# Crispy13/GeneFuseRust

Measured on NVIDIA B200. Metric: read_pairs_per_sec_matched, higher is better.
Workload: dtype u8/int64

## Files before the change

### genefuserust_b200/csrc/gf_device.cuh

```cuda
#pragma once
#include <cuda_runtime.h>
#include <stdint.h>

#define GF_GENE_PAD 2304u
#define GF_EMPTY_VAL 0xFFFFFFFFu
#define GF_HASH_MULT 0x9E3779B1u
#define GF_KIND_UNIQUE 0u
#define GF_KIND_NORMAL 1u
#define GF_KIND_HIGH 2u
#define GF_SITE_STRAND (1u << 29)
#define GF_SITE_GOFF_MASK ((1u << 29) - 1u)
#define GF_MAX_GOFF (1u << 29)
#define GF_MAX_DUPES 7

struct GfDevIndex {
    const uint4* table;
    const uint32_t* dupes;
    const uint8_t* gene_ascii;
    const uint32_t* gene_start;
    const uint32_t* gene_len;
    const uint8_t* gene_rev;
    const uint16_t* granule_contig;
    const uint32_t* g_if;
    const uint32_t* g_ir;
    const unsigned long long* filter;
    uint32_t filter_words;
    const unsigned long long* filter_multi;
    uint32_t filter_multi_words;
    uint32_t n_genes;
    uint32_t max_sites;
    uint32_t bucket_shift;
    uint32_t bucket_mask;
    int32_t major_req, minor_req, mismatch_thr, deletion_thr;
};

__device__ __forceinline__ bool gf_is_acgt_upper(uint32_t c) {
    return ((c & 0xE0u) == 0x40u) && ((0x0010008Au >> (c & 31u)) & 1u);
}
__device__ __forceinline__ uint32_t gf_code_lo(uint32_t c) { return (c >> 2) & 1u; }
__device__ __forceinline__ uint32_t gf_code_hi(uint32_t c) { return (c >> 1) & 1u; }

// ... 54 lines not shown
            c.w == GF_EMPTY_VAL;
    return v;
}
__device__ __forceinline__ uint32_t gf_table_find(const GfDevIndex& ix, uint32_t key) {
    uint32_t b = gf_home_bucket(key, ix.bucket_shift);
    for (;;) {
        uint4 a, c;
        gf_load_bucket(ix.table, b, a, c);
        bool stop;
        uint32_t v = gf_match_bucket(a, c, key, &stop);
        if (stop) return v;
        b = (b + 1) & ix.bucket_mask;
    }
}

__device__ __forceinline__ uint32_t gf_filter_word(uint32_t key, uint32_t n_words) {
    return (uint32_t)(((unsigned long long)(key * GF_HASH_MULT) * n_words) >> 32);
}
__device__ __forceinline__ void gf_filter_masks(uint32_t key, uint32_t* any_lo, uint32_t* any_hi) {
    const uint32_t g1 = key * 0xC2B2AE35u, g2 = key * 0x27D4EB2Fu;
    *any_lo = (1u << (g1 >> 27)) | (1u << ((g1 >> 22) & 31u));
    *any_hi = (1u << (g2 >> 27)) | (1u << ((g2 >> 22) & 31u));
}
__device__ __forceinline__ uint32_t gf_multi_word(uint32_t key, uint32_t n_words) {
    return (uint32_t)(((unsigned long long)(key * 0x85EBCA6Bu) * n_words) >> 32);
}
__device__ __forceinline__ unsigned long long gf_multi_mask(uint32_t key) {
    const uint32_t g = key * 0x165667B1u;
    return (1ull << (g >> 26)) | (1ull << ((g >> 20) & 63u)) | (1ull << ((g >> 14) & 63u)) | (1ull << ((g >> 8) & 63u));
}
__device__ __forceinline__ uint32_t gf_filter_sites(const GfDevIndex& ix, unsigned long long w, uint32_t key, uint32_t max_sites) {
    uint32_t al, ah;
// ... 36 lines not shown
```

### genefuserust_b200/csrc/gf_index.cu

```cuda
#include <algorithm>
#include <chrono>
#include <cstdio>
#include <cstdlib>
#include <cstring>

#include "gf_internal.h"

namespace {

constexpr int SCAN_THREADS = 256;
constexpr int SCAN_ITEMS = 8;
constexpr int SCAN_TILE = SCAN_THREADS * SCAN_ITEMS;

__global__ void k_scan_reduce(const uint32_t* __restrict__ in, uint64_t n, uint32_t* __restrict__ block_sums) {
    __shared__ uint32_t warp_sums[SCAN_THREADS / 32];
    uint64_t base = (uint64_t)blockIdx.x * SCAN_TILE;
    uint32_t s = 0;
    for (int k = 0; k < SCAN_ITEMS; k++) {
        uint64_t i = base + (uint64_t)k * SCAN_THREADS + threadIdx.x;
        if (i < n) s += in[i];
    }
    for (int o = 16; o > 0; o >>= 1) s += __shfl_down_sync(0xFFFFFFFFu, s, o);
    if ((threadIdx.x & 31) == 0) warp_sums[threadIdx.x >> 5] = s;
    __syncthreads();
// ... 170 lines not shown
    bool head = i == 0 || (uint32_t)(items[i] >> 32) != (uint32_t)(items[i - 1] >> 32);
    uint32_t c = 0;
    if (head) {
        uint32_t len = run_len_capped(items, n, i, thr + 1);
        atomicAdd(&stats[0], 1ull);
        if (len == 1) atomicAdd(&stats[1], 1ull);
        else if (len <= thr) { atomicAdd(&stats[2], 1ull); c = len; }
        else atomicAdd(&stats[3], 1ull);
    }
    ncnt[i] = c;
}
__global__ void k_build_table(const unsigned long long* __restrict__ items, uint64_t n, uint32_t thr,
                              const uint32_t* __restrict__ dupe_off, uint32_t* __restrict__ dupes,
                              unsigned long long* __restrict__ table, uint32_t bucket_shift, uint32_t bucket_mask,
                              unsigned int* __restrict__ max_disp, unsigned long long* __restrict__ filter,
                              uint32_t filter_words, unsigned long long* __restrict__ filter_multi,
                              uint32_t filter_multi_words) {
    uint64_t i = (uint64_t)blockIdx.x * blockDim.x + threadIdx.x;
    if (i >= n) return;
    uint32_t key = (uint32_t)(items[i] >> 32);
    bool head = i == 0 || key != (uint32_t)(items[i - 1] >> 32);
    if (!head) return;
    uint32_t len = run_len_capped(items, n, i, thr + 1);
    uint32_t val;
    if (len == 1) {
        val = (GF_KIND_UNIQUE << 30) | (uint32_t)(items[i] & 0x3FFFFFFFull);
    } else if (len <= thr) {
        uint32_t off = dupe_off[i];
        for (uint32_t j = 0; j < len; j++) dupes[off + j] = (uint32_t)(items[i + j] & 0x3FFFFFFFull);
        val = (GF_KIND_NORMAL << 30) | (off << 3) | len;
    } else {
        val = (GF_KIND_HIGH << 30);
    }
    if (len <= thr) {
        uint32_t al, ah;
        gf_filter_masks(key, &al, &ah);
        atomicOr(filter + gf_filter_word(key, filter_words), ((unsigned long long)ah << 32) | al);
        if (len > 1) atomicOr(filter_multi + gf_multi_word(key, filter_multi_words), gf_multi_mask(key));
    }
    unsigned long long entry = ((unsigned long long)val << 32) | key;
    uint32_t b = gf_home_bucket(key, bucket_shift);
    uint32_t disp = 0;
    for (;;) {
        unsigned long long* slot = table + 4ull * b;
        bool done = false;
        for (int s = 0; s < 4 && !done; s++) {
            if (slot[s] == ~0ull) done = atomicCAS(slot + s, ~0ull, entry) == ~0ull;
        }
        if (done) break;
        b = (b + 1) & bucket_mask;
        disp++;
    }
// ... 110 lines not shown
};
struct BuildWorkspace {
    char* base = nullptr;
    size_t cap = 0, used = 0;
    ~BuildWorkspace() { if (base) cudaFree(base); }
    cudaError_t init(size_t bytes) { cap = bytes; return cudaMalloc((void**)&base, bytes); }
    template <class T>
    T* take(size_t n) {
        size_t bytes = (n * sizeof(T) + 255) & ~(size_t)255;
        if (used + bytes > cap) return nullptr;
        T* p = reinterpret_cast<T*>(base + used);
        used += bytes;
        return p;
    }
};
__global__ void k_interleave_planes(const uint32_t* __restrict__ pl, uint32_t stride, uint32_t* __restrict__ g_if,
                                    uint32_t* __restrict__ g_ir) {
    const uint32_t w = blockIdx.x * blockDim.x + threadIdx.x;
    if (w >= stride) return;
    const uint32_t lo = pl[w], hi = pl[(size_t)stride + w], v = pl[2ull * stride + w];
    uint4* f = reinterpret_cast<uint4*>(g_if + 8ull * w);
    uint4* r = reinterpret_cast<uint4*>(g_ir + 8ull * w);
    f[0] = make_uint4(lo, hi, v, pl[3ull * stride + w]);
    f[1] = make_uint4(pl[4ull * stride + w], pl[5ull * stride + w], 0u, 0u);
    r[0] = make_uint4(lo, hi, v, pl[6ull * stride + w]);
    r[1] = make_uint4(pl[7ull * stride + w], pl[8ull * stride + w], 0u, 0u);
}

}

int gf_build_index_device(gf_index* idx, const gf_gene_span* genes, uint32_t n_genes) {
    PhaseTimer pt;
    const uint32_t thr = (uint32_t)std::max(idx->params.skip_key_dup_threshold, 2);
    cudaStream_t st = idx->stream;

    idx->n_genes = n_genes;
    idx->gene_start.resize(n_genes);
    idx->gene_len.resize(n_genes);
    std::vector<uint8_t> rev(n_genes ? n_genes : 1, 0);
    uint64_t cur = GF_GENE_PAD, gene_bytes = 0;
    for (uint32_t g = 0; g < n_genes; g++) {
// ... 115 lines not shown
    }
    if (n_dupes >= (1u << 27)) {
        gf_set_error("too many NORMAL dupe sites for the 27-bit dupe offset");
        return GF_E_LIMIT;
    }

    pt.mark("classify");
    const uint64_t n_keys = h_stats[0];
    uint32_t bucket_bits = 6;
    while ((1ull << bucket_bits) * 2 < n_keys) bucket_bits++;
    const uint64_t n_buckets = 1ull << bucket_bits;
    GF_CUDA_TRY(cudaMalloc(&idx->d_table, n_buckets * 32));
    GF_CUDA_TRY(cudaMemsetAsync(idx->d_table, 0xFF, n_buckets * 32, st));
    GF_CUDA_TRY(cudaMalloc(&idx->d_dupes, sizeof(uint32_t) * ((size_t)n_dupes + 8)));
    unsigned int* d_maxdisp = (unsigned int*)(d_stats + 6);
    const int filter_bits = 8;
    const uint32_t filter_words = (uint32_t)std::max<uint64_t>(1024, (n_keys * (uint64_t)filter_bits + 63) / 64);
    const uint32_t filter_multi_words = (uint32_t)std::max<uint64_t>(1024, (h_stats[2] * 16 + 63) / 64);
    GF_CUDA_TRY(cudaMalloc(&idx->d_filter, sizeof(unsigned long long) * ((size_t)filter_words + filter_multi_words)));
    GF_CUDA_TRY(cudaMemsetAsync(idx->d_filter, 0, sizeof(unsigned long long) * ((size_t)filter_words + filter_multi_words), st));
    unsigned long long* d_filter_multi = (unsigned long long*)idx->d_filter + filter_words;
    if (n_items) {
        const unsigned cb = (unsigned)((n_items + 255) / 256);
        k_build_table<<<cb, 256, 0, st>>>(d_items, n_items, thr, d_doff, (uint32_t*)idx->d_dupes,
                                          (unsigned long long*)idx->d_table, 32 - bucket_bits,
                                          (uint32_t)(n_buckets - 1), d_maxdisp, (unsigned long long*)idx->d_filter,
                                          filter_words, d_filter_multi, filter_multi_words);
        GF_CUDA_TRY(cudaGetLastError());
    }
    unsigned int h_maxdisp = 0;
    GF_CUDA_TRY(cudaMemcpyAsync(&h_maxdisp, d_maxdisp, sizeof(unsigned int), cudaMemcpyDeviceToHost, st));
    GF_CUDA_TRY(cudaStreamSynchronize(st));

    pt.mark("table + filter");
    idx->dev.table = (const uint4*)idx->d_table;
    idx->dev.dupes = (const uint32_t*)idx->d_dupes;
    idx->dev.gene_ascii = (const uint8_t*)idx->d_gene_ascii;
    idx->dev.gene_start = (const uint32_t*)idx->d_gene_start;
    idx->dev.gene_len = (const uint32_t*)idx->d_gene_len;
    idx->dev.gene_rev = (const uint8_t*)idx->d_gene_rev;
    idx->dev.n_genes = n_genes;
    idx->dev.max_sites = thr;
    idx->dev.bucket_shift = 32 - bucket_bits;
    idx->dev.bucket_mask = (uint32_t)(n_buckets - 1);
    idx->dev.major_req = idx->params.major_gene_key_requirement;
    idx->dev.minor_req = idx->params.minor_gene_key_requirement;
    idx->dev.mismatch_thr = idx->params.mismatch_threshold;
    idx->dev.deletion_thr = idx->params.deletion_threshold;
    idx->dev.filter = (const unsigned long long*)idx->d_filter;
    idx->dev.filter_words = filter_words;
    idx->dev.filter_multi = d_filter_multi;
    idx->dev.filter_multi_words = filter_multi_words;

    const uint32_t n_pw = (uint32_t)((arena_len + 31) / 32);
    const size_t plane_stride = ((size_t)n_pw + 72 + 7) & ~(size_t)7;
    DevTmp tmp_planes;
    GF_CUDA_TRY(cudaMalloc(&tmp_planes.p, sizeof(uint32_t) * plane_stride * 9));
    GF_CUDA_TRY(cudaMemsetAsync(tmp_planes.p, 0, sizeof(uint32_t) * plane_stride * 9, st));
    GF_CUDA_TRY(cudaMalloc(&idx->d_planes, sizeof(uint32_t) * plane_stride * 16));
    uint32_t* pl = (uint32_t*)tmp_planes.p;
    uint32_t* gi = (uint32_t*)idx->d_planes;
    k_gene_planes<<<(n_pw + 255) / 256, 256, 0, st>>>((const uint8_t*)idx->d_gene_ascii, arena_len, n_pw, pl,
                                                      pl + plane_stride, pl + 2 * plane_stride);
    k_window_class<<<ex_blocks, EX_THREADS, 0, st>>>(idx->dev, (const uint8_t*)idx->d_gene_ascii, arena_len,
                                                     pl + 3 * plane_stride, pl + 6 * plane_stride,
                                                     (uint32_t)plane_stride);
    idx->dev.g_if = gi;
    idx->dev.g_ir = gi + 8 * plane_stride;
    k_interleave_planes<<<(unsigned)((plane_stride + 255) / 256), 256, 0, st>>>(pl, (uint32_t)plane_stride, gi, gi + 8 * plane_stride);
    GF_CUDA_TRY(cudaGetLastError());
    GF_CUDA_TRY(cudaEventRecord(e1, st));
    GF_CUDA_TRY(cudaStreamSynchronize(st));
    float ms = 0;
    GF_CUDA_TRY(cudaEventElapsedTime(&ms, e0, e1));

    pt.mark("gene planes + window class");
    gf_index_info& inf = idx->info;
    inf.n_sites = n_items;
    inf.n_keys = n_keys;
    inf.n_unique = h_stats[1];
    inf.n_normal = h_stats[2];
    inf.n_high = h_stats[3];
    inf.table_slots = n_buckets * 4;
    inf.table_bytes = n_buckets * 32;
    inf.max_displacement = h_maxdisp;
    inf.gene_bytes = gene_bytes;
    inf.device_bytes = n_buckets * 32 + sizeof(uint32_t) * ((size_t)n_dupes + 8) + arena_len + 9ull * (n_genes + 1) +
                       sizeof(uint32_t) * plane_stride * 16 + sizeof(unsigned long long) * ((size_t)filter_words + filter_multi_words);
    inf.build_ms = ms;
    return GF_OK;
}

int gf_lookup_device(gf_index* idx, const uint32_t* kmers, uint64_t n, gf_lookup* out) {
    if (n == 0) return GF_OK;
    DevTmp k, o;
    GF_CUDA_TRY(cudaMalloc(&k.p, sizeof(uint32_t) * n));
    GF_CUDA_TRY(cudaMalloc(&o.p, sizeof(gf_lookup) * n));
    GF_CUDA_TRY(cudaMemcpyAsync(k.p, kmers, sizeof(uint32_t) * n, cudaMemcpyHostToDevice, idx->stream));
    k_lookup<<<(unsigned)((n + 127) / 128), 128, 0, idx->stream>>>(idx->dev, (const uint32_t*)k.p, n, (gf_lookup*)o.p);
    GF_CUDA_TRY(cudaGetLastError());
    GF_CUDA_TRY(cudaMemcpyAsync(out, o.p, sizeof(gf_lookup) * n, cudaMemcpyDeviceToHost, idx->stream));
    GF_CUDA_TRY(cudaStreamSynchronize(idx->stream));
    return GF_OK;
// ... 2 lines not shown
```

### genefuserust_b200/csrc/gf_map.cu

```cuda
#include <climits>
#include <cstdlib>
#include <cstdio>

#include "gf_internal.h"
#include "gf_swar.cuh"

namespace {

#define FULL 0xFFFFFFFFu
using swar::zero_bytes;

__device__ __forceinline__ uint32_t fsr(const uint32_t* plane, uint32_t bitpos) {
    uint32_t w = bitpos >> 5;
    return __funnelshift_r(plane[w], plane[w + 1], bitpos & 31u);
}
__device__ __forceinline__ uint32_t lowmask(int nbits) {
    return nbits >= 32 ? 0xFFFFFFFFu : ((1u << nbits) - 1u);
}
__device__ __forceinline__ bool record_ok(uint64_t s, uint64_t e, uint64_t base, uint64_t bytes, int max_len) {
    if (e < s || e - s > (uint64_t)max_len || s < base) return false;
    return bytes == 0 || (s - base <= bytes && e - s <= bytes - (s - base));
}

template <int MAXW>
struct ScreenWarp {
    uint32_t r1lo[MAXW + 1], r1hi[MAXW + 1], r1v[MAXW + 1], r1n[MAXW + 1], q1hi[MAXW + 1], q1lo[MAXW + 1];
    uint32_t c2lo[MAXW + 1], c2hi[MAXW + 1], c2v[MAXW + 1], c2n[MAXW + 1], q2hi[MAXW + 1], q2lo[MAXW + 1];
    uint32_t xlo[MAXW + 1], xhi[MAXW + 1], xv[MAXW + 1];
    uint32_t mlo[2 * MAXW + 2], mhi[2 * MAXW + 2], mv[2 * MAXW + 2];
    uint32_t rlo[2 * MAXW + 2], rhi[2 * MAXW + 2], rv[2 * MAXW + 2];
    uint32_t glo[2 * MAXW + 3], ghi[2 * MAXW + 3], gv[2 * MAXW + 3], gc[3][2 * MAXW + 3];
    uint32_t eq[2 * MAXW + 2], hit[2 * MAXW + 2];
    uint16_t others[32 * MAXW + 32];
    uint32_t f2lo[MAXW + 1], f2hi[MAXW + 1], f2v[MAXW + 1];
    uint32_t sp[6][MAXW + 4];
};

__device__ __forceinline__ uint32_t gather4(uint32_t t) {
    return ((t * 0x01020408u) >> 24) & 0xFu;
}
__device__ __forceinline__ void classify4(uint32_t x, bool ci, uint32_t* lo, uint32_t* hi, uint32_t* v) {
    const uint32_t xu = ci ? (x & 0xDFDFDFDFu) : x;
    const uint32_t t = (xu >> 1) & 0x03030303u;
    const uint32_t u = t | (t >> 4);
    const uint32_t sel = (u & 0xFFu) | ((u >> 8) & 0xFF00u);
    const uint32_t expect = __byte_perm(0x47544341u, 0u, sel);
// ... 214 lines not shown
    x &= x >> 2;
    x &= x >> 4;
    x &= x >> 8;
    return (uint32_t)x;
}
__device__ __forceinline__ unsigned long long make_policy_keep() {
    unsigned long long pol;
    asm volatile("createpolicy.fractional.L2::evict_last.b64 %0, 1.0;" : "=l"(pol));
    return pol;
}
__device__ __forceinline__ unsigned long long ldg_filter(const unsigned long long* p, unsigned long long pol) {
    unsigned long long v;
    asm volatile("ld.global.nc.L1::no_allocate.L2::cache_hint.u64 %0, [%1], %2;" : "=l"(v) : "l"(p), "l"(pol));
    return v;
}

template <int MAXW>
__device__ __forceinline__ bool screen_sequence2(const GfDevIndex& ix, ScreenWarp<MAXW>& S, const uint32_t* lo,
                                                 const uint32_t* hi, const uint32_t* v, int len, int need_total,
                                                 int need_minor, unsigned long long* probes) {
    const uint32_t lane = gf_lane();
    const int nprobe = len >= 16 ? ((len - 16) >> 1) + 1 : 0;
    *probes += (unsigned long long)nprobe;
    if (need_total <= 0 || need_minor <= 0) return nprobe > 0 || need_total <= 0;
    if (nprobe == 0) return false;
    const int nch = (len + 31) >> 5;
    const unsigned long long pol = make_policy_keep();

    uint32_t seed_val = GF_EMPTY_VAL;
    int seed_i = 0;
    {
        int i = (int)(((long long)(lane & 7u) * nprobe) >> 3) * 2;
        bool ok = lane < 8 && (fsr(v, (uint32_t)i) & 0xFFFFu) == 0xFFFFu;
        uint32_t key = ((fsr(hi, (uint32_t)i) & 0xFFFFu) << 16) | (fsr(lo, (uint32_t)i) & 0xFFFFu);
        bool present = false;
        if (ok) present = gf_filter_sites(ix, ldg_filter(ix.filter + gf_filter_word(key, ix.filter_words), pol), key, 2u) == 1u;
        uint32_t pm = __ballot_sync(FULL, present);
        while (pm) {
            int src = __ffs(pm) - 1;
            pm &= pm - 1;
            uint32_t k = __shfl_sync(FULL, key, src);
            uint32_t val = gf_table_find(ix, k);
            if (val != GF_EMPTY_VAL && (val >> 30) == GF_KIND_UNIQUE) {
                seed_val = val;
                seed_i = __shfl_sync(FULL, i, src);
                break;
            }
        }
    }

    int T = 0, c_d = 0;
// ... 12 lines not shown
                if (k < nch) {
                    int pos = len - 32 * k - 32;
                    if (pos >= 0) { a = fsr(lo, (uint32_t)pos); b = fsr(hi, (uint32_t)pos); c = fsr(v, (uint32_t)pos); }
                    else if (pos > -32) { a = lo[0] << (-pos); b = hi[0] << (-pos); c = v[0] << (-pos); }
                    a = __brev(a); b = __brev(b); c = __brev(c);
                    a = (a ^ c) & c;
                }
                S.rlo[k] = a; S.rhi[k] = b; S.rv[k] = c;
            }
            plo = S.rlo; phi = S.rhi; pv = S.rv;
            D = goff + (uint32_t)seed_i - (uint32_t)len + 1u;
            if (len & 1) parity = 0xAAAAAAAAu;
            __syncwarp();
        }
        const uint32_t wbase = D >> 5, sh = D & 31u;
        const uint4* gi = reinterpret_cast<const uint4*>(rc ? ix.g_ir : ix.g_if);
        for (int k = (int)lane; k <= nch + 1; k += 32) {
            const uint4 a = __ldg(gi + 2ull * (wbase + k)), b = __ldg(gi + 2ull * (wbase + k) + 1);
            S.glo[k] = a.x; S.ghi[k] = a.y; S.gv[k] = a.z;
            S.gc[0][k] = a.w; S.gc[1][k] = b.x; S.gc[2][k] = b.y;
        }
        __syncwarp();
        for (int k = (int)lane; k <= nch; k += 32) {
            uint32_t e = 0;
            if (k < nch) {
                uint32_t glo = __funnelshift_r(S.glo[k], S.glo[k + 1], sh);
                uint32_t ghi = __funnelshift_r(S.ghi[k], S.ghi[k + 1], sh);
                uint32_t gvv = __funnelshift_r(S.gv[k], S.gv[k + 1], sh);
                e = ~((plo[k] ^ glo) | (phi[k] ^ ghi)) & pv[k] & gvv;
            }
            S.eq[k] = e;
        }
        __syncwarp();
        int c = 0, t = 0;
        for (int k = (int)lane; k < nch; k += 32) {
            uint32_t m = run16(S.eq[k], S.eq[k + 1]) & parity;
            uint32_t c0 = __funnelshift_r(S.gc[0][k], S.gc[0][k + 1], sh) & m;
            uint32_t c1 = __funnelshift_r(S.gc[1][k], S.gc[1][k + 1], sh) & m;
            uint32_t c2 = __funnelshift_r(S.gc[2][k], S.gc[2][k + 1], sh) & m;
            uint32_t h = c0 | c1 | c2;
            S.hit[k] = h;
            c += __popc(h);
            t += __popc(c0) + 2 * __popc(c1) + 4 * __popc(c2);
        }
        c_d = (int)__reduce_add_sync(FULL, (unsigned)c);
        T = (int)__reduce_add_sync(FULL, (unsigned)t);
    }
    __syncwarp();

    int t_local = 0;
    if (seed_val == GF_EMPTY_VAL) {
        for (int j0 = 0; j0 < nprobe; j0 += 64) {
            uint32_t key[2];
            unsigned long long w[2];
            bool ok[2];
#pragma unroll
            for (int u = 0; u < 2; u++) {
                int j = j0 + 32 * u + (int)lane;
                uint32_t off = 2u * (uint32_t)min(j, nprobe - 1);
                ok[u] = j < nprobe && (fsr(pv, off) & 0xFFFFu) == 0xFFFFu;
                key[u] = ((fsr(phi, off) & 0xFFFFu) << 16) | (fsr(plo, off) & 0xFFFFu);
                w[u] = 0;
                if (ok[u]) w[u] = ldg_filter(ix.filter + gf_filter_word(key[u], ix.filter_words), pol);
            }
#pragma unroll
            for (int u = 0; u < 2; u++)
                if (ok[u]) t_local += (int)gf_filter_sites(ix, w[u], key[u], ix.max_sites);
        }
    } else {
        int total = 0;
        for (int k0 = 0; k0 < nch; k0 += 32) {
            int k = k0 + (int)lane;
            uint32_t om = 0;
            if (k < nch) om = run16(pv[k], pv[k + 1]) & parity & ~S.hit[k];
            if (__ballot_sync(FULL, om != 0u) == 0u) continue;
            int cnt = __popc(om);
            int incl = cnt;
            for (int o = 1; o < 32; o <<= 1) {
// ... 2 lines not shown
            }
            int pos = total + incl - cnt;
            while (om) {
                int b = __ffs(om) - 1;
                om &= om - 1;
                S.others[pos++] = (uint16_t)(32 * k + b);
            }
            total += __shfl_sync(FULL, incl, 31);
        }
        __syncwarp();
        for (int j = (int)lane; j - (int)lane < total; j += 32) {
            if (j < total) {
                uint32_t off = S.others[j];
                uint32_t kk = ((fsr(phi, off) & 0xFFFFu) << 16) | (fsr(plo, off) & 0xFFFFu);
                uint32_t key = rc ? gf_key_revcomp(kk) : kk;
                t_local += (int)gf_filter_sites(ix, ldg_filter(ix.filter + gf_filter_word(key, ix.filter_words), pol), key,
                                                ix.max_sites);
            }
        }
    }
    T += (int)__reduce_add_sync(FULL, (unsigned)t_local);
    return T >= need_total && (T - c_d) >= need_minor;
}

#include "gf_screen_tpp.cuh"
#include "gf_screen_split.cuh"

template <int MAXW, bool PAIRED>
__global__ void __launch_bounds__(256, 3) k_screen(ScreenParams P) {
    extern __shared__ __align__(16) unsigned char smem_raw[];
    ScreenWarp<MAXW>* Sall = reinterpret_cast<ScreenWarp<MAXW>*>(smem_raw);
    const uint32_t lane = gf_lane();
// ... 1075 lines not shown
```

### genefuserust_b200/csrc/gf_screen_split.cuh

```cuda
#pragma once

namespace split {

using tpp::Col;
using tpp::Lay;

#ifndef GF_STORE_STREAMING
#define GF_STORE_STREAMING 1
#endif
template <class T>
__device__ __forceinline__ T st_ld(const T* p) {
#if GF_STORE_STREAMING
    return __ldcs(p);
#else
    return *p;
#endif
}
template <class T>
__device__ __forceinline__ void st_st(T* p, T v) {
#if GF_STORE_STREAMING
    __stcs(p, v);
#else
    *p = v;
#endif
// ... 227 lines not shown
                    key[2 * j + 1] = (phi[j] & 0xFFFF0000u) | (plo[j] >> 16);
                    if (32 * j + 16 <= len && (pv[j] & 0xFFFFu) == 0xFFFFu) okm |= 1u << (2 * j);
                    if (32 * j + 32 <= len && (pv[j] >> 16) == 0xFFFFu) okm |= 2u << (2 * j);
                }
                if (okm) {
                    const uint32_t t0 = (uint32_t)__ffs(okm) - 1u;
                    uint32_t k0 = key[0];
#pragma unroll
                    for (int t = 1; t < 8; t++) if (t0 == (uint32_t)t) k0 = key[t];
                    tpp::prefetch_l2(P.ix.table + 2ull * gf_home_bucket(k0, P.ix.bucket_shift));
                }
                unsigned long long fw[8];
#pragma unroll
                for (int t = 0; t < 8; t++) {
                    fw[t] = 0;
                    if ((okm >> t) & 1u) fw[t] = ldg_filter(P.ix.filter + gf_filter_word(key[t], P.ix.filter_words), pol);
                }
                uint32_t pm = 0;
#pragma unroll
                for (int t = 0; t < 8; t++) {
                    uint32_t al, ah;
                    gf_filter_masks(key[t], &al, &ah);
                    const uint32_t wl = (uint32_t)fw[t], wh = (uint32_t)(fw[t] >> 32);
                    if (((okm >> t) & 1u) && (wl & al) == al && (wh & ah) == ah) pm |= 1u << t;
                }
                seed_i = pm | (okm << 8);
                while (pm) {
                    const int t = __ffs(pm) - 1;
                    pm &= pm - 1u;
                    uint32_t kt = key[0];
#pragma unroll
// ... 29 lines not shown

struct ClassParams {
    GfDevIndex ix;
    SeqStore st;
    uint2* survivors;
    uint32_t survivors_cap;
    GfMapCounters* counters;
    int need_total, need_minor;
};
__device__ __forceinline__ void push_survivor(const ClassParams& P, const uint4& m) {
    uint32_t slot = atomicAdd(&P.counters->n_survivors, 1u);
    if (slot < P.survivors_cap) P.survivors[slot] = make_uint2(m.x, m.y);
    else atomicOr(&P.counters->error_flags, 2u);
}
template <int W>
__global__ void __launch_bounds__(256) k_scan(ClassParams P) {
    constexpr int NW = SL<W>::NW;
    const unsigned long long pol = make_policy_keep();
    const GfDevIndex& ix = P.ix;
    const int need_major = P.need_total - P.need_minor;
    const uint32_t n = P.st.counters[2];
    for (uint32_t t = blockIdx.x * blockDim.x + threadIdx.x; t < n; t += gridDim.x * blockDim.x) {
        const uint32_t s = st_ld(&P.st.list[P.st.cap - 1u - t]);
        const uint4 m = st_ld(&P.st.meta[s]);
        const int len = (int)m.z, nch = (len + 31) >> 5;
        const uint32_t* col = slot_words<W>(P.st, s);
        uint32_t lo = st_ld(&col[0]), hi = st_ld(&col[(size_t)NW * 32]), v = st_ld(&col[(size_t)2 * NW * 32]);
        const uint32_t pre = st_ld(&P.st.seed[s]).y, pre_valid = (pre >> 8) & 0xFFu;
        int Pn = __popc(pre & 0xFFu);
        bool dead = false;
#pragma unroll 1
        for (int k = 0; k < nch && !dead; k++) {
            const uint32_t nlo = st_ld(&col[(size_t)(k + 1) * 32]), nhi = st_ld(&col[(size_t)(NW + k + 1) * 32]), nv = st_ld(&col[(size_t)(2 * NW + k + 1) * 32]);
            uint32_t om = run16(v, nv) & 0x55555555u;
            if (k < 4) om &= ~0x00010001u;
            const int beyond = len - 16 - 32 * (k + 1);
            const int rem_after = (beyond >= 0 ? (beyond >> 1) + 1 : 0) - (k < 3 ? __popc(pre_valid >> (2 * (k + 1))) : 0);
            while (om) {
                uint32_t key[4];
                unsigned long long w[4];
                bool ok[4];
#pragma unroll
                for (int u = 0; u < 4; u++) {
                    ok[u] = om != 0u;
                    const uint32_t b = ok[u] ? (uint32_t)(__ffs(om) - 1) : 0u;
                    om &= om - 1u;
                    key[u] = ((__funnelshift_r(hi, nhi, b) & 0xFFFFu) << 16) | (__funnelshift_r(lo, nlo, b) & 0xFFFFu);
                    w[u] = 0;
                    if (ok[u]) w[u] = ldg_filter(ix.filter + gf_filter_word(key[u], ix.filter_words), pol);
                }
#pragma unroll
                for (int u = 0; u < 4; u++)
                    if (ok[u] && gf_filter_present(w[u], key[u])) Pn++;
                const int rem = __popc(om) + rem_after;
                if (P.need_total > 0 && Pn + rem < need_major) { dead = true; break; }
            }
            lo = nlo; hi = nhi; v = nv;
        }
        if (P.need_total <= 0 || (!dead && Pn >= need_major && 2 * Pn >= P.need_total)) push_survivor(P, m);
    }
}

struct GeneWord { uint32_t lo, hi, v, a, b, c, pad0, pad1; };
__device__ __forceinline__ GeneWord ldg_gene_word(const uint32_t* base, uint32_t w, unsigned long long pol) {
    GeneWord g;
    asm volatile("ld.global.nc.L2::cache_hint.v8.u32 {%0,%1,%2,%3,%4,%5,%6,%7}, [%8], %9;"
                 : "=r"(g.lo), "=r"(g.hi), "=r"(g.v), "=r"(g.a), "=r"(g.b), "=r"(g.c), "=r"(g.pad0), "=r"(g.pad1)
                 : "l"(base + 8ull * w), "l"(pol));
    return g;
}
constexpr int DIAG_Q = 128;
template <int W>
__global__ void __launch_bounds__(256, 5) k_diag(ClassParams P) {
    constexpr int NW = SL<W>::NW;
    __shared__ uint32_t q_lo0[8][DIAG_Q], q_lo1[8][DIAG_Q], q_hi0[8][DIAG_Q], q_hi1[8][DIAG_Q], q_om[8][DIAG_Q], q_meta[8][DIAG_Q];
    __shared__ int t_sh[8][32];
    __shared__ unsigned q_cnt[8];
    const uint32_t lane = gf_lane(), wib = threadIdx.x >> 5;
    const unsigned long long pol = make_policy_keep();
    const GfDevIndex& ix = P.ix;
    auto flush = [&]() {
        __syncwarp();
        const int total = (int)q_cnt[wib];
#pragma unroll 2
        for (int base = 0; base < total; base += 2) {
            const int e = base + (int)(lane >> 4);
            if (e < total) {
                const uint32_t om = q_om[wib][e], meta = q_meta[wib][e];
                const uint32_t b = 2u * (lane & 15u) + ((meta >> 9) & 1u);
                if ((om >> b) & 1u) {
                    const uint32_t kk = ((__funnelshift_r(q_hi0[wib][e], q_hi1[wib][e], b) & 0xFFFFu) << 16) |
                                        (__funnelshift_r(q_lo0[wib][e], q_lo1[wib][e], b) & 0xFFFFu);
                    const uint32_t key = ((meta >> 8) & 1u) ? gf_key_revcomp(kk) : kk;
                    if (gf_filter_present(ldg_filter(ix.filter + gf_filter_word(key, ix.filter_words), pol), key))
                        atomicAdd(&t_sh[wib][meta & 31u], 2);
                }
            }
        }
        __syncwarp();
        if (lane == 0) q_cnt[wib] = 0;
        __syncwarp();
    };
    const uint32_t n = P.st.counters[1];
    for (uint32_t t0 = blockIdx.x * blockDim.x + (threadIdx.x & ~31u); t0 < n; t0 += gridDim.x * blockDim.x) {
        const bool have = t0 + lane < n;
        const uint32_t s = have ? st_ld(&P.st.list[t0 + lane]) : 0u;
        const uint4 m = have ? st_ld(&P.st.meta[s]) : make_uint4(0, 0, 0, 0);
        const uint2 sd = have ? st_ld(&P.st.seed[s]) : make_uint2(0, 0);
        const int len = (int)m.z, nch = have ? (len + 31) >> 5 : 0;
        const uint32_t* col = slot_words<W>(P.st, s);
        const bool rc = (sd.x & GF_SITE_STRAND) != 0;
        const uint32_t goff = sd.x & GF_SITE_GOFF_MASK;
        const uint32_t D = rc ? goff + sd.y - (uint32_t)len + 1u : goff - sd.y;
        const uint32_t parity = (rc && (len & 1)) ? 0xAAAAAAAAu : 0x55555555u;
        const uint32_t wbase = D >> 5, sh = D & 31u;
        const uint32_t* gi = rc ? ix.g_ir : ix.g_if;
        t_sh[wib][lane] = 0;
        if (lane == 0) q_cnt[wib] = 0;
        __syncwarp();
        auto read_chunk = [&](int k, uint32_t* lo, uint32_t* hi, uint32_t* v) {
            if (k >= nch) { *lo = *hi = *v = 0; return; }
            if (!rc) { *lo = st_ld(&col[(size_t)k * 32]); *hi = st_ld(&col[(size_t)(NW + k) * 32]); *v = st_ld(&col[(size_t)(2 * NW + k) * 32]); return; }
            int pos = len - 32 * k - 32;
            uint32_t a, b, cc;
            if (pos >= 0) { a = fs_col(col, 0, (uint32_t)pos); b = fs_col(col, NW, (uint32_t)pos); cc = fs_col(col, 2 * NW, (uint32_t)pos); }
            else { a = st_ld(&col[0]) << (-pos); b = st_ld(&col[(size_t)NW * 32]) << (-pos); cc = st_ld(&col[(size_t)2 * NW * 32]) << (-pos); }
            uint32_t vv = __brev(cc);
            *v = vv;
            *lo = ~__brev(a) & vv;
            *hi = __brev(b);
        };
        GeneWord g0 = {0, 0, 0, 0, 0, 0, 0, 0};
        uint32_t lo_cur = 0, hi_cur = 0, v_cur = 0, e_cur = 0, cnt_a = 0, cnt_b = 0, cnt_c = 0;
        if (have) {
            g0 = ldg_gene_word(gi, wbase, pol);
            const GeneWord g1 = ldg_gene_word(gi, wbase + 1, pol);
            read_chunk(0, &lo_cur, &hi_cur, &v_cur);
            e_cur = ~((lo_cur ^ __funnelshift_r(g0.lo, g1.lo, sh)) | (hi_cur ^ __funnelshift_r(g0.hi, g1.hi, sh))) & v_cur &
                    __funnelshift_r(g0.v, g1.v, sh);
            cnt_a = __funnelshift_r(g0.a, g1.a, sh); cnt_b = __funnelshift_r(g0.b, g1.b, sh); cnt_c = __funnelshift_r(g0.c, g1.c, sh);
            g0 = g1;
        }
        int T = 0, c_d = 0;
        const int max_nch = (int)__reduce_max_sync(FULL, (unsigned)nch);
#pragma unroll 1
        for (int k = 0; k < max_nch; k++) {
            if (k < nch) {
                uint32_t nlo, nhi, nv;
                read_chunk(k + 1, &nlo, &nhi, &nv);
                uint32_t e_nxt = 0, na = 0, nb = 0, nc = 0;
                if (k + 1 < nch) {
                    const GeneWord g1 = ldg_gene_word(gi, wbase + k + 2, pol);
                    e_nxt = ~((nlo ^ __funnelshift_r(g0.lo, g1.lo, sh)) | (nhi ^ __funnelshift_r(g0.hi, g1.hi, sh))) & nv &
                            __funnelshift_r(g0.v, g1.v, sh);
                    na = __funnelshift_r(g0.a, g1.a, sh); nb = __funnelshift_r(g0.b, g1.b, sh); nc = __funnelshift_r(g0.c, g1.c, sh);
                    g0 = g1;
                }
                uint32_t mm = run16(e_cur, e_nxt) & parity;
                uint32_t c0 = cnt_a & mm, c1 = cnt_b & mm, c2 = cnt_c & mm;
                uint32_t hit = c0 | c1 | c2;
                c_d += __popc(hit);
                T += __popc(hit) + __popc(c1 | c2);
                uint32_t om = run16(v_cur, nv) & parity & ~hit;
                e_cur = e_nxt; cnt_a = na; cnt_b = nb; cnt_c = nc;
                if (om) {
                    const unsigned pos = atomicAdd(&q_cnt[wib], 1u);
                    q_lo0[wib][pos] = lo_cur; q_lo1[wib][pos] = nlo; q_hi0[wib][pos] = hi_cur; q_hi1[wib][pos] = nhi;
                    q_om[wib][pos] = om;
                    q_meta[wib][pos] = lane | (rc ? 0x100u : 0u) | ((parity & 1u) ? 0u : 0x200u);
                }
                v_cur = nv; lo_cur = nlo; hi_cur = nhi;
            }
            __syncwarp();
            if (q_cnt[wib] > (unsigned)(DIAG_Q - 32)) flush();
        }
        flush();
        T += t_sh[wib][lane];
        if (have && (P.need_total <= 0 || P.need_minor <= 0 || (T >= P.need_total && (T - c_d) >= P.need_minor))) push_survivor(P, m);
        __syncwarp();
// ... 5 lines not shown
```

Baseline: 1.988 billion.

## Pair-blocked bloom filter and merged forward/reverse gene plane layout

Restructures the bloom filter into 32-byte sectors where k-mers sharing a core land in adjacent words, so k_scan can test two k-mers (offset by 2) with one 16-byte load. Each key is inserted into both phase-A and phase-B slots, and filter bits per key drop to 6. The forward and reverse gene class planes are merged into one 32-byte record holding precomputed OR'd masks, which halves the plane memory and lets the scan do fewer funnelshifts. Also adds a launch-bounds occupancy hint and defers the meta load. The filter's false-positive characteristics change, which may alter how many candidates survive screening.

Result: faster. 2.014 billion (median of 6 runs) (+1.3%).

```diff
diff --git a/genefuserust_b200/csrc/gf_device.cuh b/genefuserust_b200/csrc/gf_device.cuh
--- a/genefuserust_b200/csrc/gf_device.cuh
+++ b/genefuserust_b200/csrc/gf_device.cuh
@@ -21,10 +21,9 @@
     const uint32_t* gene_len;
     const uint8_t* gene_rev;
     const uint16_t* granule_contig;
-    const uint32_t* g_if;
-    const uint32_t* g_ir;
+    const uint32_t* g_planes;
     const unsigned long long* filter;
-    uint32_t filter_words;
+    uint32_t filter_sectors;
     const unsigned long long* filter_multi;
     uint32_t filter_multi_words;
     uint32_t n_genes;
@@ -109,8 +108,18 @@
     }
 }
 
-__device__ __forceinline__ uint32_t gf_filter_word(uint32_t key, uint32_t n_words) {
-    return (uint32_t)(((unsigned long long)(key * GF_HASH_MULT) * n_words) >> 32);
+#define GF_FILTER_PHASE_A 0u
+#define GF_FILTER_PHASE_B 1u
+__device__ __forceinline__ uint32_t gf_filter_core(uint32_t key, uint32_t phase) {
+    const uint32_t s = 2u - 2u * phase;
+    return ((key >> s) & 0x3FFFu) | ((key >> (s + 2u)) & 0x0FFFC000u);
+}
+__device__ __forceinline__ uint32_t gf_filter_half(uint32_t core, uint32_t n_sectors) {
+    const uint32_t sector = (uint32_t)(((unsigned long long)(core * 0x7FEB352Du) * n_sectors) >> 32);
+    return 2u * sector + ((core * 0xCC9E2D51u) >> 31);
+}
+__device__ __forceinline__ uint32_t gf_filter_index(uint32_t key, uint32_t phase, uint32_t n_sectors) {
+    return 2u * gf_filter_half(gf_filter_core(key, phase), n_sectors) + phase;
 }
 __device__ __forceinline__ void gf_filter_masks(uint32_t key, uint32_t* any_lo, uint32_t* any_hi) {
     const uint32_t g1 = key * 0xC2B2AE35u, g2 = key * 0x27D4EB2Fu;
diff --git a/genefuserust_b200/csrc/gf_index.cu b/genefuserust_b200/csrc/gf_index.cu
--- a/genefuserust_b200/csrc/gf_index.cu
+++ b/genefuserust_b200/csrc/gf_index.cu
@@ -208,7 +208,7 @@
                               const uint32_t* __restrict__ dupe_off, uint32_t* __restrict__ dupes,
                               unsigned long long* __restrict__ table, uint32_t bucket_shift, uint32_t bucket_mask,
                               unsigned int* __restrict__ max_disp, unsigned long long* __restrict__ filter,
-                              uint32_t filter_words, unsigned long long* __restrict__ filter_multi,
+                              uint32_t filter_sectors, unsigned long long* __restrict__ filter_multi,
                               uint32_t filter_multi_words) {
     uint64_t i = (uint64_t)blockIdx.x * blockDim.x + threadIdx.x;
     if (i >= n) return;
@@ -229,7 +229,9 @@
     if (len <= thr) {
         uint32_t al, ah;
         gf_filter_masks(key, &al, &ah);
-        atomicOr(filter + gf_filter_word(key, filter_words), ((unsigned long long)ah << 32) | al);
+        const unsigned long long bits = ((unsigned long long)ah << 32) | al;
+        atomicOr(filter + gf_filter_index(key, GF_FILTER_PHASE_A, filter_sectors), bits);
+        atomicOr(filter + gf_filter_index(key, GF_FILTER_PHASE_B, filter_sectors), bits);
         if (len > 1) atomicOr(filter_multi + gf_multi_word(key, filter_multi_words), gf_multi_mask(key));
     }
     unsigned long long entry = ((unsigned long long)val << 32) | key;
@@ -370,17 +372,15 @@
         return p;
     }
 };
-__global__ void k_interleave_planes(const uint32_t* __restrict__ pl, uint32_t stride, uint32_t* __restrict__ g_if,
-                                    uint32_t* __restrict__ g_ir) {
+__global__ void k_interleave_planes(const uint32_t* __restrict__ pl, uint32_t stride, uint32_t* __restrict__ g) {
     const uint32_t w = blockIdx.x * blockDim.x + threadIdx.x;
     if (w >= stride) return;
     const uint32_t lo = pl[w], hi = pl[(size_t)stride + w], v = pl[2ull * stride + w];
-    uint4* f = reinterpret_cast<uint4*>(g_if + 8ull * w);
-    uint4* r = reinterpret_cast<uint4*>(g_ir + 8ull * w);
-    f[0] = make_uint4(lo, hi, v, pl[3ull * stride + w]);
-    f[1] = make_uint4(pl[4ull * stride + w], pl[5ull * stride + w], 0u, 0u);
-    r[0] = make_uint4(lo, hi, v, pl[6ull * stride + w]);
-    r[1] = make_uint4(pl[7ull * stride + w], pl[8ull * stride + w], 0u, 0u);
+    const uint32_t f0 = pl[3ull * stride + w], f12 = pl[4ull * stride + w] | pl[5ull * stride + w];
+    const uint32_t r0 = pl[6ull * stride + w], r12 = pl[7ull * stride + w] | pl[8ull * stride + w];
+    uint4* e = reinterpret_cast<uint4*>(g + 8ull * w);
+    e[0] = make_uint4(lo, hi, v, f0 | f12);
+    e[1] = make_uint4(f12, r0 | r12, r12, 0u);
 }
 
 }
@@ -526,8 +526,9 @@
     GF_CUDA_TRY(cudaMemsetAsync(idx->d_table, 0xFF, n_buckets * 32, st));
     GF_CUDA_TRY(cudaMalloc(&idx->d_dupes, sizeof(uint32_t) * ((size_t)n_dupes + 8)));
     unsigned int* d_maxdisp = (unsigned int*)(d_stats + 6);
-    const int filter_bits = 8;
-    const uint32_t filter_words = (uint32_t)std::max<uint64_t>(1024, (n_keys * (uint64_t)filter_bits + 63) / 64);
+    const int filter_bits = 6;
+    const uint32_t filter_sectors = (uint32_t)std::max<uint64_t>(256, (2 * n_keys * (uint64_t)filter_bits + 255) / 256);
+    const uint32_t filter_words = 4 * filter_sectors;
     const uint32_t filter_multi_words = (uint32_t)std::max<uint64_t>(1024, (h_stats[2] * 16 + 63) / 64);
     GF_CUDA_TRY(cudaMalloc(&idx->d_filter, sizeof(unsigned long long) * ((size_t)filter_words + filter_multi_words)));
     GF_CUDA_TRY(cudaMemsetAsync(idx->d_filter, 0, sizeof(unsigned long long) * ((size_t)filter_words + filter_multi_words), st));
@@ -537,7 +538,7 @@
         k_build_table<<<cb, 256, 0, st>>>(d_items, n_items, thr, d_doff, (uint32_t*)idx->d_dupes,
                                           (unsigned long long*)idx->d_table, 32 - bucket_bits,
                                           (uint32_t)(n_buckets - 1), d_maxdisp, (unsigned long long*)idx->d_filter,
-                                          filter_words, d_filter_multi, filter_multi_words);
+                                          filter_sectors, d_filter_multi, filter_multi_words);
         GF_CUDA_TRY(cudaGetLastError());
     }
     unsigned int h_maxdisp = 0;
@@ -560,7 +561,7 @@
     idx->dev.mismatch_thr = idx->params.mismatch_threshold;
     idx->dev.deletion_thr = idx->params.deletion_threshold;
     idx->dev.filter = (const unsigned long long*)idx->d_filter;
-    idx->dev.filter_words = filter_words;
+    idx->dev.filter_sectors = filter_sectors;
     idx->dev.filter_multi = d_filter_multi;
     idx->dev.filter_multi_words = filter_multi_words;
 
@@ -569,7 +570,7 @@
     DevTmp tmp_planes;
     GF_CUDA_TRY(cudaMalloc(&tmp_planes.p, sizeof(uint32_t) * plane_stride * 9));
     GF_CUDA_TRY(cudaMemsetAsync(tmp_planes.p, 0, sizeof(uint32_t) * plane_stride * 9, st));
-    GF_CUDA_TRY(cudaMalloc(&idx->d_planes, sizeof(uint32_t) * plane_stride * 16));
+    GF_CUDA_TRY(cudaMalloc(&idx->d_planes, sizeof(uint32_t) * plane_stride * 8));
     uint32_t* pl = (uint32_t*)tmp_planes.p;
     uint32_t* gi = (uint32_t*)idx->d_planes;
     k_gene_planes<<<(n_pw + 255) / 256, 256, 0, st>>>((const uint8_t*)idx->d_gene_ascii, arena_len, n_pw, pl,
@@ -577,9 +578,8 @@
     k_window_class<<<ex_blocks, EX_THREADS, 0, st>>>(idx->dev, (const uint8_t*)idx->d_gene_ascii, arena_len,
                                                      pl + 3 * plane_stride, pl + 6 * plane_stride,
                                                      (uint32_t)plane_stride);
-    idx->dev.g_if = gi;
-    idx->dev.g_ir = gi + 8 * plane_stride;
-    k_interleave_planes<<<(unsigned)((plane_stride + 255) / 256), 256, 0, st>>>(pl, (uint32_t)plane_stride, gi, gi + 8 * plane_stride);
+    idx->dev.g_planes = gi;
+    k_interleave_planes<<<(unsigned)((plane_stride + 255) / 256), 256, 0, st>>>(pl, (uint32_t)plane_stride, gi);
     GF_CUDA_TRY(cudaGetLastError());
     GF_CUDA_TRY(cudaEventRecord(e1, st));
     GF_CUDA_TRY(cudaStreamSynchronize(st));
@@ -598,7 +598,7 @@
     inf.max_displacement = h_maxdisp;
     inf.gene_bytes = gene_bytes;
     inf.device_bytes = n_buckets * 32 + sizeof(uint32_t) * ((size_t)n_dupes + 8) + arena_len + 9ull * (n_genes + 1) +
-                       sizeof(uint32_t) * plane_stride * 16 + sizeof(unsigned long long) * ((size_t)filter_words + filter_multi_words);
+                       sizeof(uint32_t) * plane_stride * 8 + sizeof(unsigned long long) * ((size_t)filter_words + filter_multi_words);
     inf.build_ms = ms;
     return GF_OK;
 }
diff --git a/genefuserust_b200/csrc/gf_map.cu b/genefuserust_b200/csrc/gf_map.cu
--- a/genefuserust_b200/csrc/gf_map.cu
+++ b/genefuserust_b200/csrc/gf_map.cu
@@ -29,7 +29,7 @@
     uint32_t xlo[MAXW + 1], xhi[MAXW + 1], xv[MAXW + 1];
     uint32_t mlo[2 * MAXW + 2], mhi[2 * MAXW + 2], mv[2 * MAXW + 2];
     uint32_t rlo[2 * MAXW + 2], rhi[2 * MAXW + 2], rv[2 * MAXW + 2];
-    uint32_t glo[2 * MAXW + 3], ghi[2 * MAXW + 3], gv[2 * MAXW + 3], gc[3][2 * MAXW + 3];
+    uint32_t glo[2 * MAXW + 3], ghi[2 * MAXW + 3], gv[2 * MAXW + 3], gc[2][2 * MAXW + 3];
     uint32_t eq[2 * MAXW + 2], hit[2 * MAXW + 2];
     uint16_t others[32 * MAXW + 32];
     uint32_t f2lo[MAXW + 1], f2hi[MAXW + 1], f2v[MAXW + 1];
@@ -274,6 +274,12 @@
     asm volatile("ld.global.nc.L1::no_allocate.L2::cache_hint.u64 %0, [%1], %2;" : "=l"(v) : "l"(p), "l"(pol));
     return v;
 }
+__device__ __forceinline__ uint4 ldg_filter_half(const unsigned long long* filter, uint32_t half, unsigned long long pol) {
+    uint4 v;
+    asm volatile("ld.global.nc.L1::no_allocate.L2::cache_hint.v4.u32 {%0,%1,%2,%3}, [%4], %5;"
+                 : "=r"(v.x), "=r"(v.y), "=r"(v.z), "=r"(v.w) : "l"(filter + 2ull * half), "l"(pol));
+    return v;
+}
 
 template <int MAXW>
 __device__ __forceinline__ bool screen_sequence2(const GfDevIndex& ix, ScreenWarp<MAXW>& S, const uint32_t* lo,
@@ -294,7 +300,9 @@
         bool ok = lane < 8 && (fsr(v, (uint32_t)i) & 0xFFFFu) == 0xFFFFu;
         uint32_t key = ((fsr(hi, (uint32_t)i) & 0xFFFFu) << 16) | (fsr(lo, (uint32_t)i) & 0xFFFFu);
         bool present = false;
-        if (ok) present = gf_filter_sites(ix, ldg_filter(ix.filter + gf_filter_word(key, ix.filter_words), pol), key, 2u) == 1u;
+        if (ok)
+            present = gf_filter_sites(ix, ldg_filter(ix.filter + gf_filter_index(key, GF_FILTER_PHASE_A, ix.filter_sectors), pol),
+                                      key, 2u) == 1u;
         uint32_t pm = __ballot_sync(FULL, present);
         while (pm) {
             int src = __ffs(pm) - 1;
@@ -337,11 +345,11 @@
             __syncwarp();
         }
         const uint32_t wbase = D >> 5, sh = D & 31u;
-        const uint4* gi = reinterpret_cast<const uint4*>(rc ? ix.g_ir : ix.g_if);
+        const uint4* gi = reinterpret_cast<const uint4*>(ix.g_planes);
         for (int k = (int)lane; k <= nch + 1; k += 32) {
             const uint4 a = __ldg(gi + 2ull * (wbase + k)), b = __ldg(gi + 2ull * (wbase + k) + 1);
             S.glo[k] = a.x; S.ghi[k] = a.y; S.gv[k] = a.z;
-            S.gc[0][k] = a.w; S.gc[1][k] = b.x; S.gc[2][k] = b.y;
+            S.gc[0][k] = rc ? b.y : a.w; S.gc[1][k] = rc ? b.z : b.x;
         }
         __syncwarp();
         for (int k = (int)lane; k <= nch; k += 32) {
@@ -358,13 +366,11 @@
         int c = 0, t = 0;
         for (int k = (int)lane; k < nch; k += 32) {
             uint32_t m = run16(S.eq[k], S.eq[k + 1]) & parity;
-            uint32_t c0 = __funnelshift_r(S.gc[0][k], S.gc[0][k + 1], sh) & m;
-            uint32_t c1 = __funnelshift_r(S.gc[1][k], S.gc[1][k + 1], sh) & m;
-            uint32_t c2 = __funnelshift_r(S.gc[2][k], S.gc[2][k + 1], sh) & m;
-            uint32_t h = c0 | c1 | c2;
+            const uint32_t h = __funnelshift_r(S.gc[0][k], S.gc[0][k + 1], sh) & m;
+            const uint32_t h2 = __funnelshift_r(S.gc[1][k], S.gc[1][k + 1], sh) & m;
             S.hit[k] = h;
             c += __popc(h);
-            t += __popc(c0) + 2 * __popc(c1) + 4 * __popc(c2);
+            t += __popc(h) + __popc(h2);
         }
         c_d = (int)__reduce_add_sync(FULL, (unsigned)c);
         T = (int)__reduce_add_sync(FULL, (unsigned)t);
@@ -384,7 +390,7 @@
                 ok[u] = j < nprobe && (fsr(pv, off) & 0xFFFFu) == 0xFFFFu;
                 key[u] = ((fsr(phi, off) & 0xFFFFu) << 16) | (fsr(plo, off) & 0xFFFFu);
                 w[u] = 0;
-                if (ok[u]) w[u] = ldg_filter(ix.filter + gf_filter_word(key[u], ix.filter_words), pol);
+                if (ok[u]) w[u] = ldg_filter(ix.filter + gf_filter_index(key[u], GF_FILTER_PHASE_A, ix.filter_sectors), pol);
             }
 #pragma unroll
             for (int u = 0; u < 2; u++)
@@ -417,8 +423,8 @@
                 uint32_t off = S.others[j];
                 uint32_t kk = ((fsr(phi, off) & 0xFFFFu) << 16) | (fsr(plo, off) & 0xFFFFu);
                 uint32_t key = rc ? gf_key_revcomp(kk) : kk;
-                t_local += (int)gf_filter_sites(ix, ldg_filter(ix.filter + gf_filter_word(key, ix.filter_words), pol), key,
-                                                ix.max_sites);
+                const unsigned long long w = ldg_filter(ix.filter + gf_filter_index(key, GF_FILTER_PHASE_A, ix.filter_sectors), pol);
+                t_local += (int)gf_filter_sites(ix, w, key, ix.max_sites);
             }
         }
     }
diff --git a/genefuserust_b200/csrc/gf_screen_split.cuh b/genefuserust_b200/csrc/gf_screen_split.cuh
--- a/genefuserust_b200/csrc/gf_screen_split.cuh
+++ b/genefuserust_b200/csrc/gf_screen_split.cuh
@@ -265,7 +265,8 @@
 #pragma unroll
                 for (int t = 0; t < 8; t++) {
                     fw[t] = 0;
-                    if ((okm >> t) & 1u) fw[t] = ldg_filter(P.ix.filter + gf_filter_word(key[t], P.ix.filter_words), pol);
+                    if ((okm >> t) & 1u)
+                        fw[t] = ldg_filter(P.ix.filter + gf_filter_index(key[t], GF_FILTER_PHASE_A, P.ix.filter_sectors), pol);
                 }
                 uint32_t pm = 0;
 #pragma unroll
@@ -325,7 +326,7 @@
     else atomicOr(&P.counters->error_flags, 2u);
 }
 template <int W>
-__global__ void __launch_bounds__(256) k_scan(ClassParams P) {
+__global__ void __launch_bounds__(256, 6) k_scan(ClassParams P) {
     constexpr int NW = SL<W>::NW;
     const unsigned long long pol = make_policy_keep();
     const GfDevIndex& ix = P.ix;
@@ -333,8 +334,7 @@
     const uint32_t n = P.st.counters[2];
     for (uint32_t t = blockIdx.x * blockDim.x + threadIdx.x; t < n; t += gridDim.x * blockDim.x) {
         const uint32_t s = st_ld(&P.st.list[P.st.cap - 1u - t]);
-        const uint4 m = st_ld(&P.st.meta[s]);
-        const int len = (int)m.z, nch = (len + 31) >> 5;
+        const int len = (int)st_ld(&P.st.meta[s].z), nch = (len + 31) >> 5;
         const uint32_t* col = slot_words<W>(P.st, s);
         uint32_t lo = st_ld(&col[0]), hi = st_ld(&col[(size_t)NW * 32]), v = st_ld(&col[(size_t)2 * NW * 32]);
         const uint32_t pre = st_ld(&P.st.seed[s]).y, pre_valid = (pre >> 8) & 0xFFu;
@@ -347,36 +347,47 @@
             if (k < 4) om &= ~0x00010001u;
             const int beyond = len - 16 - 32 * (k + 1);
             const int rem_after = (beyond >= 0 ? (beyond >> 1) + 1 : 0) - (k < 3 ? __popc(pre_valid >> (2 * (k + 1))) : 0);
+            constexpr int NF = 3;
             while (om) {
-                uint32_t key[4];
-                unsigned long long w[4];
-                bool ok[4];
-#pragma unroll
-                for (int u = 0; u < 4; u++) {
+                uint32_t bb[NF];
+                uint4 w[NF];
+                bool ok[NF], two[NF];
+#pragma unroll
+                for (int u = 0; u < NF; u++) {
                     ok[u] = om != 0u;
                     const uint32_t b = ok[u] ? (uint32_t)(__ffs(om) - 1) : 0u;
                     om &= om - 1u;
-                    key[u] = ((__funnelshift_r(hi, nhi, b) & 0xFFFFu) << 16) | (__funnelshift_r(lo, nlo, b) & 0xFFFFu);
-                    w[u] = 0;
-                    if (ok[u]) w[u] = ldg_filter(ix.filter + gf_filter_word(key[u], ix.filter_words), pol);
-                }
-#pragma unroll
-                for (int u = 0; u < 4; u++)
-                    if (ok[u] && gf_filter_present(w[u], key[u])) Pn++;
+                    two[u] = ((om >> b) & 4u) != 0u;
+                    om &= ~((two[u] ? 4u : 0u) << b);
+                    bb[u] = b;
+                    const uint32_t key = ((__funnelshift_r(hi, nhi, b) & 0xFFFFu) << 16) | (__funnelshift_r(lo, nlo, b) & 0xFFFFu);
+                    w[u] = make_uint4(0, 0, 0, 0);
+                    if (ok[u])
+                        w[u] = ldg_filter_half(ix.filter, gf_filter_half(gf_filter_core(key, GF_FILTER_PHASE_A), ix.filter_sectors), pol);
+                }
+#pragma unroll
+                for (int u = 0; u < NF; u++) {
+                    const uint32_t b = bb[u];
+                    const uint32_t ka = ((__funnelshift_r(hi, nhi, b) & 0xFFFFu) << 16) | (__funnelshift_r(lo, nlo, b) & 0xFFFFu);
+                    const uint32_t kb =
+                        ((__funnelshift_r(hi, nhi, b + 2u) & 0xFFFFu) << 16) | (__funnelshift_r(lo, nlo, b + 2u) & 0xFFFFu);
+                    if (ok[u] && gf_filter_present(((unsigned long long)w[u].y << 32) | w[u].x, ka)) Pn++;
+                    if (two[u] && gf_filter_present(((unsigned long long)w[u].w << 32) | w[u].z, kb)) Pn++;
+                }
                 const int rem = __popc(om) + rem_after;
                 if (P.need_total > 0 && Pn + rem < need_major) { dead = true; break; }
             }
             lo = nlo; hi = nhi; v = nv;
         }
-        if (P.need_total <= 0 || (!dead && Pn >= need_major && 2 * Pn >= P.need_total)) push_survivor(P, m);
+        if (P.need_total <= 0 || (!dead && Pn >= need_major && 2 * Pn >= P.need_total)) push_survivor(P, st_ld(&P.st.meta[s]));
     }
 }
 
-struct GeneWord { uint32_t lo, hi, v, a, b, c, pad0, pad1; };
+struct GeneWord { uint32_t lo, hi, v, f1, f2, r1, r2, pad; };
 __device__ __forceinline__ GeneWord ldg_gene_word(const uint32_t* base, uint32_t w, unsigned long long pol) {
     GeneWord g;
     asm volatile("ld.global.nc.L2::cache_hint.v8.u32 {%0,%1,%2,%3,%4,%5,%6,%7}, [%8], %9;"
-                 : "=r"(g.lo), "=r"(g.hi), "=r"(g.v), "=r"(g.a), "=r"(g.b), "=r"(g.c), "=r"(g.pad0), "=r"(g.pad1)
+                 : "=r"(g.lo), "=r"(g.hi), "=r"(g.v), "=r"(g.f1), "=r"(g.f2), "=r"(g.r1), "=r"(g.r2), "=r"(g.pad)
                  : "l"(base + 8ull * w), "l"(pol));
     return g;
 }
@@ -402,8 +413,10 @@
                 if ((om >> b) & 1u) {
                     const uint32_t kk = ((__funnelshift_r(q_hi0[wib][e], q_hi1[wib][e], b) & 0xFFFFu) << 16) |
                                         (__funnelshift_r(q_lo0[wib][e], q_lo1[wib][e], b) & 0xFFFFu);
-                    const uint32_t key = ((meta >> 8) & 1u) ? gf_key_revcomp(kk) : kk;
-                    if (gf_filter_present(ldg_filter(ix.filter + gf_filter_word(key, ix.filter_words), pol), key))
+                    const uint32_t rcm = (meta >> 8) & 1u;
+                    const uint32_t key = rcm ? gf_key_revcomp(kk) : kk;
+                    const uint32_t phase = (lane & 1u) ^ rcm;
+                    if (gf_filter_present(ldg_filter(ix.filter + gf_filter_index(key, phase, ix.filter_sectors), pol), key))
                         atomicAdd(&t_sh[wib][meta & 31u], 2);
                 }
             }
@@ -425,7 +438,7 @@
         const uint32_t D = rc ? goff + sd.y - (uint32_t)len + 1u : goff - sd.y;
         const uint32_t parity = (rc && (len & 1)) ? 0xAAAAAAAAu : 0x55555555u;
         const uint32_t wbase = D >> 5, sh = D & 31u;
-        const uint32_t* gi = rc ? ix.g_ir : ix.g_if;
+        const uint32_t* gi = ix.g_planes;
         t_sh[wib][lane] = 0;
         if (lane == 0) q_cnt[wib] = 0;
         __syncwarp();
@@ -442,14 +455,15 @@
             *hi = __brev(b);
         };
         GeneWord g0 = {0, 0, 0, 0, 0, 0, 0, 0};
-        uint32_t lo_cur = 0, hi_cur = 0, v_cur = 0, e_cur = 0, cnt_a = 0, cnt_b = 0, cnt_c = 0;
+        uint32_t lo_cur = 0, hi_cur = 0, v_cur = 0, e_cur = 0, cnt_1 = 0, cnt_2 = 0;
         if (have) {
             g0 = ldg_gene_word(gi, wbase, pol);
             const GeneWord g1 = ldg_gene_word(gi, wbase + 1, pol);
             read_chunk(0, &lo_cur, &hi_cur, &v_cur);
             e_cur = ~((lo_cur ^ __funnelshift_r(g0.lo, g1.lo, sh)) | (hi_cur ^ __funnelshift_r(g0.hi, g1.hi, sh))) & v_cur &
                     __funnelshift_r(g0.v, g1.v, sh);
-            cnt_a = __funnelshift_r(g0.a, g1.a, sh); cnt_b = __funnelshift_r(g0.b, g1.b, sh); cnt_c = __funnelshift_r(g0.c, g1.c, sh);
+            cnt_1 = __funnelshift_r(rc ? g0.r1 : g0.f1, rc ? g1.r1 : g1.f1, sh);
+            cnt_2 = __funnelshift_r(rc ? g0.r2 : g0.f2, rc ? g1.r2 : g1.f2, sh);
             g0 = g1;
         }
         int T = 0, c_d = 0;
@@ -459,21 +473,21 @@
             if (k < nch) {
                 uint32_t nlo, nhi, nv;
                 read_chunk(k + 1, &nlo, &nhi, &nv);
-                uint32_t e_nxt = 0, na = 0, nb = 0, nc = 0;
+                uint32_t e_nxt = 0, n1 = 0, n2 = 0;
                 if (k + 1 < nch) {
                     const GeneWord g1 = ldg_gene_word(gi, wbase + k + 2, pol);
                     e_nxt = ~((nlo ^ __funnelshift_r(g0.lo, g1.lo, sh)) | (nhi ^ __funnelshift_r(g0.hi, g1.hi, sh))) & nv &
                             __funnelshift_r(g0.v, g1.v, sh);
-                    na = __funnelshift_r(g0.a, g1.a, sh); nb = __funnelshift_r(g0.b, g1.b, sh); nc = __funnelshift_r(g0.c, g1.c, sh);
+                    n1 = __funnelshift_r(rc ? g0.r1 : g0.f1, rc ? g1.r1 : g1.f1, sh);
+                    n2 = __funnelshift_r(rc ? g0.r2 : g0.f2, rc ? g1.r2 : g1.f2, sh);
                     g0 = g1;
                 }
                 uint32_t mm = run16(e_cur, e_nxt) & parity;
-                uint32_t c0 = cnt_a & mm, c1 = cnt_b & mm, c2 = cnt_c & mm;
-                uint32_t hit = c0 | c1 | c2;
+                const uint32_t hit = cnt_1 & mm;
                 c_d += __popc(hit);
-                T += __popc(hit) + __popc(c1 | c2);
+                T += __popc(hit) + __popc(cnt_2 & mm);
                 uint32_t om = run16(v_cur, nv) & parity & ~hit;
-                e_cur = e_nxt; cnt_a = na; cnt_b = nb; cnt_c = nc;
+                e_cur = e_nxt; cnt_1 = n1; cnt_2 = n2;
                 if (om) {
                     const unsigned pos = atomicAdd(&q_cnt[wib], 1u);
                     q_lo0[wib][pos] = lo_cur; q_lo1[wib][pos] = nlo; q_hi0[wib][pos] = hi_cur; q_hi1[wib][pos] = nhi;
```
